# pyannote/pyannote-audio

Measured on AMD Instinct MI355X. Metric: audio-hours/sec (real-time factor) for speaker-diarization-3.1 pipeline, higher is better.
Workload: dtype f32

## Files before the change

pyannote-audio_amd/csrc/emb_resnet.hip:

```cpp
#include "common.h"

namespace pa {

constexpr int STEM_TS = 64;
constexpr int STEM_LD = STEM_TS + 3;

__global__ __launch_bounds__(256) void k_stem(const float* __restrict__ fb, int T, int F,
                                              const float* __restrict__ w9,
                                              const float* __restrict__ shift,
                                              float* __restrict__ out) {
  extern __shared__ float xs[];
  const int b = blockIdx.y, t0 = blockIdx.x * STEM_TS;
  const int tid = threadIdx.x;
  for (int i = tid; i < 2 * STEM_LD; i += 256) xs[(i < STEM_LD ? 0 : (F + 1) * STEM_LD - STEM_LD) + i] = 0.f;
  const int n = (STEM_TS + 2) * F;
  for (int i0 = 0; i0 < n; i0 += 8 * 256) {
    float v[8];
#pragma unroll
    for (int k = 0; k < 8; ++k) {
      const int i = i0 + tid + 256 * k;
      const int tt = i / F, ff = i - tt * F, t = t0 + tt - 1;
      v[k] = (i < n && t >= 0 && t < T) ? fb[((long)b * T + t) * F + ff] : 0.f;
    }
#pragma unroll
    for (int k = 0; k < 8; ++k) {
      const int i = i0 + tid + 256 * k;
      const int tt = i / F, ff = i - tt * F;
      if (i < n) xs[(ff + 1) * STEM_LD + tt] = v[k];
    }
  }
  const int q4 = (tid & 7) * 4, pl = tid >> 3;
  float w[9][4], sh[4];
#pragma unroll
  for (int k = 0; k < 9; ++k)
#pragma unroll
    for (int c = 0; c < 4; ++c) w[k][c] = w9[k * 32 + q4 + c];
#pragma unroll
  for (int c = 0; c < 4; ++c) sh[c] = shift[q4 + c];
  __syncthreads();
  float x0[2][3], x1[2][3], x2[2][3];
#pragma unroll
  for (int h = 0; h < 2; ++h)
#pragma unroll
    for (int dt = 0; dt < 3; ++dt) {
      x0[h][dt] = xs[0 * STEM_LD + pl + 32 * h + dt];
      x1[h][dt] = xs[1 * STEM_LD + pl + 32 * h + dt];
    }
  const bool ok0 = t0 + pl < T, ok1 = t0 + pl + 32 < T;
  float* o = out + ((long)b * F * T + t0 + pl) * 32 + q4;
  for (int f = 0; f < F; ++f) {
#pragma unroll
    for (int h = 0; h < 2; ++h)
#pragma unroll
      for (int dt = 0; dt < 3; ++dt) x2[h][dt] = xs[(f + 2) * STEM_LD + pl + 32 * h + dt];
    float* of = o + (long)f * T * 32;
#pragma unroll
    for (int h = 0; h < 2; ++h) {
      float acc[4];
#pragma unroll
      for (int c = 0; c < 4; ++c) acc[c] = 0.f;
#pragma unroll
      for (int dt = 0; dt < 3; ++dt)
#pragma unroll
        for (int c = 0; c < 4; ++c) acc[c] = fmaf(x0[h][dt], w[dt][c], acc[c]);
#pragma unroll
      for (int dt = 0; dt < 3; ++dt)
#pragma unroll
        for (int c = 0; c < 4; ++c) acc[c] = fmaf(x1[h][dt], w[3 + dt][c], acc[c]);
#pragma unroll
      for (int dt = 0; dt < 3; ++dt)
#pragma unroll
        for (int c = 0; c < 4; ++c) acc[c] = fmaf(x2[h][dt], w[6 + dt][c], acc[c]);
      float4 o4;
      o4.x = fmaxf(acc[0] + sh[0], 0.f);
      o4.y = fmaxf(acc[1] + sh[1], 0.f);
      o4.z = fmaxf(acc[2] + sh[2], 0.f);
      o4.w = fmaxf(acc[3] + sh[3], 0.f);
      if (h == 0 ? ok0 : ok1) *reinterpret_cast<float4*>(of + 32 * 32 * h) = o4;
    }
#pragma unroll
    for (int h = 0; h < 2; ++h)
#pragma unroll
      for (int dt = 0; dt < 3; ++dt) {
        x0[h][dt] = x1[h][dt];
        x1[h][dt] = x2[h][dt];
      }
  }
}

constexpr int CB = 16;
constexpr int CLD = CB + 4;

template <int S, int TH, int TWT>
struct ConvGeom {
  static constexpr int TW = 32 * TWT;
  static constexpr int PH = (TH - 1) * S + 3;
  static constexpr int PW = (TW - 1) * S + 3;
  static constexpr int PWH = ((TW + 1 + 3) / 8) * 8 + 4;
  static constexpr int PATCH = S == 1 ? PH * PW * CLD : PH * 2 * PWH * CLD;
};

template <int S, int TH, int TWT, int BN, bool HAS_R>
__global__ __launch_bounds__(256, 2) void k_conv3x3(const float* __restrict__ X, int H, int W, int CIN,
                                                    const float* __restrict__ Wg,
                                                    const float* __restrict__ shift,
                                                    const float* __restrict__ R, float* __restrict__ Y,
                                                    int Ho, int Wo, int COUT, int relu, int tiles_w,
                                                    int tiles_hw, int n_tiles, int total_tiles, int xranges,
                                                    int* __restrict__ counters) {
  using G = ConvGeom<S, TH, TWT>;
  constexpr int MT = TH * TWT;
  constexpr int MPW = MT / 4;
  constexpr int NT = BN / 32;
  static_assert(MT % 4 == 0, "M-tiles must split over 4 waves");
  extern __shared__ __attribute__((aligned(16))) float smem[];
  float* patch = smem;
  float* wts = smem + G::PATCH;

  const int tid = threadIdx.x, lane = tid & 63, wv = tid >> 6;
  const int li = lane & 31, kh = lane >> 5;
  constexpr int NPF4 = G::PH * G::PW * (CB / 4);
  constexpr int NP = (NPF4 + 255) / 256;
  constexpr int NWF4 = 9 * BN * (CB / 4);
  constexpr int NW = (NWF4 + 255) / 256;
  constexpr int OOB = (int)0x80000000;

  struct Tile {
    int b, n0, y0, x0;
  };
  const int num_pb = total_tiles / n_tiles;
  auto pair_of = [&](int t) {
    return xranges ? (t & 7) * ((num_pb + 7) >> 3) + (t >> 3) / n_tiles : ((t >> 3) / n_tiles) * 8 + (t & 7);
  };
  auto decode = [&](int t) {
    Tile q;
    const int pb = pair_of(t);
    q.n0 = (((t >> 3) % n_tiles)) * BN;
    const int pix = pb % tiles_hw;
    q.b = pb / tiles_hw;
    q.y0 = (pix / tiles_w) * TH;
    q.x0 = (pix % tiles_w) * G::TW;
    return q;
  };
  auto resolve = [&](const TileQueue& tqq, int r) {
    for (;;) {
      const int t = tq_resolve(tqq, r);
      if (t < 0 || pair_of(t) < num_pb) return t;
      r = tq_claim_own(tqq);
    }
  };
  u32x4 rp[NP], rw[NW];
  constexpr bool HOIST = S == 2;
  struct Offs {
    int p[NP];
  };
  int offw[NW];
#pragma unroll
  for (int e = 0; e < NW; ++e) {
    const int i = tid + 256 * e;
    const int c4 = i & 3, rn = i >> 2;
    const int tap = rn / BN, n = rn % BN;
    offw[e] = (NWF4 % 256 == 0 || i < NWF4) ? ((tap * COUT + n) * CIN + 4 * c4) * 4 : OOB;
  }
  auto tile_offsets = [&](const Tile& q, Offs& o) {
#pragma unroll
    for (int e = 0; e < NP; ++e) {
      const int i = tid + 256 * e;
      const int c4 = i & 3, pp = i >> 2;
      const int py = pp / G::PW, px = pp % G::PW;
      const int iy = q.y0 * S - 1 + py, ix = q.x0 * S - 1 + px;
      o.p[e] = ((NPF4 % 256 == 0 || i < NPF4) && iy >= 0 && iy < H && ix >= 0 && ix < W)
                   ? ((iy * W + ix) * CIN + 4 * c4) * 4
                   : OOB;
    }
  };
  auto gload = [&](const Tile& q, const Offs& o, int c0) {
    const __amdgpu_buffer_rsrc_t xsrd = __builtin_amdgcn_make_buffer_rsrc(
        const_cast<float*>(X + (long)q.b * H * W * CIN), 0, H * W * CIN * 4, 0x00020000);
    const __amdgpu_buffer_rsrc_t wsrd = __builtin_amdgcn_make_buffer_rsrc(
        const_cast<float*>(Wg + (long)q.n0 * CIN), 0, (9 * COUT - q.n0) * CIN * 4, 0x00020000);
    Offs here;
    if (!HOIST) tile_offsets(q, here);
#pragma unroll
    for (int e = 0; e < NP; ++e)
      rp[e] = __builtin_amdgcn_raw_buffer_load_b128(xsrd, HOIST ? o.p[e] : here.p[e], c0 * 4, 0);
#pragma unroll
    for (int e = 0; e < NW; ++e) rw[e] = __builtin_amdgcn_raw_buffer_load_b128(wsrd, offw[e], c0 * 4, 0);
  };
  auto lstore = [&]() {
#pragma unroll
    for (int e = 0; e < NP; ++e) {
      const int i = tid + 256 * e;
      const int c4 = i & 3, pp = i >> 2;
      const int py = pp / G::PW, px = pp % G::PW;
      int off;
      if (S == 1) off = pp * CLD + 4 * c4;
      else off = ((py * 2 + (px & 1)) * G::PWH + (px >> 1)) * CLD + 4 * c4;
      if (NPF4 % 256 == 0 || i < NPF4) *reinterpret_cast<u32x4*>(patch + off) = rp[e];
    }
#pragma unroll
    for (int e = 0; e < NW; ++e) {
      const int i = tid + 256 * e;
      if (NWF4 % 256 == 0 || i < NWF4)
        *reinterpret_cast<u32x4*>(wts + (i >> 2) * CLD + 4 * (i & 3)) = rw[e];
    }
  };

  __shared__ int s_next;
  const TileQueue tq{counters, (int)(blockIdx.x & 7), ((num_pb + 7) >> 3) * n_tiles};
  if (tid == 0) s_next = resolve(tq, tq_claim_own(tq));
  __syncthreads();
  int t = s_next;
  if (t < 0) {
    if (tid == 0) tq_done(tq, gridDim.x);
    return;
  }
  Tile cur = decode(t);
  Offs oc, on;
  if (HOIST) tile_offsets(cur, oc);
  on = oc;
  gload(cur, oc, 0);
  for (;;) {
    int ahead = 0;
    if (tid == 0) ahead = tq_claim_own(tq);
    int tn = -1;
    f32x16 acc[MPW][NT];
#pragma unroll
    for (int i = 0; i < MPW; ++i)
#pragma unroll
      for (int j = 0; j < NT; ++j)
#pragma unroll
        for (int r = 0; r < 16; ++r) acc[i][j][r] = 0.f;
    Tile nxt = cur;

    for (int c0 = 0; c0 < CIN; c0 += CB) {
      __syncthreads();
      lstore();
      if (c0 == 0 && tid == 0) s_next = resolve(tq, ahead);
      __syncthreads();
      if (c0 == 0) {
        tn = s_next;
        if (tn >= 0) {
          nxt = decode(tn);
          if (HOIST) tile_offsets(nxt, on);
        }
      }
      if (c0 + CB < CIN) gload(cur, oc, c0 + CB);
      else if (tn >= 0) gload(nxt, on, 0);
      float4 af[1][MPW][2], bf[1][NT][2];
      auto load_tap = [&](int tap, float4 (&a)[MPW][2], float4 (&bq)[NT][2]) {
        const int dy = tap / 3, dx = tap % 3;
#pragma unroll
        for (int i = 0; i < MPW; ++i) {
          const int mt = wv * MPW + i;
          const int yy = mt / TWT, xt = mt % TWT;
          int off;
          if (S == 1) off = ((yy + dy) * G::PW + 32 * xt + li + dx) * CLD;
          else off = (((yy * 2 + dy) * 2 + (dx & 1)) * G::PWH + 32 * xt + li + (dx >> 1)) * CLD;
          a[i][0] = *reinterpret_cast<const float4*>(patch + off + kh * 8);
          a[i][1] = *reinterpret_cast<const float4*>(patch + off + kh * 8 + 4);
        }
#pragma unroll
        for (int j = 0; j < NT; ++j) {
          const int off = (tap * BN + 32 * j + li) * CLD + kh * 8;
          bq[j][0] = *reinterpret_cast<const float4*>(wts + off);
          bq[j][1] = *reinterpret_cast<const float4*>(wts + off + 4);
        }
      };
      auto mfma_tap = [&](const float4 (&a)[MPW][2], const float4 (&bq)[NT][2]) {
#pragma unroll
        for (int h = 0; h < 2; ++h)
#pragma unroll
          for (int i = 0; i < MPW; ++i)
#pragma unroll
            for (int j = 0; j < NT; ++j) {
              acc[i][j] = MFMA32(a[i][h].x, bq[j][h].x, acc[i][j]);
              acc[i][j] = MFMA32(a[i][h].y, bq[j][h].y, acc[i][j]);
              acc[i][j] = MFMA32(a[i][h].z, bq[j][h].z, acc[i][j]);
              acc[i][j] = MFMA32(a[i][h].w, bq[j][h].w, acc[i][j]);
            }
      };
#pragma unroll 1
      for (int dy = 0; dy < 3; ++dy)
#pragma unroll
        for (int dx = 0; dx < 3; ++dx) {
          load_tap(dy * 3 + dx, af[0], bf[0]);
          mfma_tap(af[0], bf[0]);
        }
    }
    {
      const __amdgpu_buffer_rsrc_t ysrd = __builtin_amdgcn_make_buffer_rsrc(
          Y + (long)cur.b * Ho * Wo * COUT, 0, Ho * Wo * COUT * 4, 0x00020000);
      const __amdgpu_buffer_rsrc_t rsrd = __builtin_amdgcn_make_buffer_rsrc(
          const_cast<float*>(HAS_R ? R + (long)cur.b * Ho * Wo * COUT : Y), 0,
          Ho * Wo * COUT * 4, 0x00020000);
      constexpr int NG = MPW * NT;
      int off[2][16];
      float rv[2][16];
      auto goffs = [&](int g, int* o) {
        const int i = g / NT, j = g % NT;
        const int mt = wv * MPW + i;
        const int y = cur.y0 + mt / TWT, xbase = cur.x0 + 32 * (mt % TWT) + 4 * kh;
        const int n = cur.n0 + 32 * j + li;
#pragma unroll
        for (int r = 0; r < 16; ++r) {
          const int x = xbase + (r & 3) + 8 * (r >> 2);
          o[r] = (y < Ho && x < Wo) ? ((y * Wo + x) * COUT + n) * 4 : OOB;
        }
      };
      auto gres = [&](const int* o, float* v) {
        if (HAS_R) {
#pragma unroll
          for (int r = 0; r < 16; ++r)
            v[r] = __builtin_bit_cast(float, __builtin_amdgcn_raw_buffer_load_b32(rsrd, o[r], 0, 0));
        } else {
#pragma unroll
          for (int r = 0; r < 16; ++r) v[r] = 0.f;
        }
      };
      goffs(0, off[0]);
      gres(off[0], rv[0]);
#pragma unroll
      for (int g = 0; g < NG; ++g) {
        if (g + 1 < NG) {
          goffs(g + 1, off[(g + 1) & 1]);
          gres(off[(g + 1) & 1], rv[(g + 1) & 1]);
        }
        const int i = g / NT, j = g % NT;
        const float sh = shift[cur.n0 + 32 * j + li];
#pragma unroll
        for (int r = 0; r < 16; ++r) {
          float v = acc[i][j][r] + sh + rv[g & 1][r];
          if (relu) v = fmaxf(v, 0.f);
          __builtin_amdgcn_raw_buffer_store_b32(__builtin_bit_cast(unsigned int, v), ysrd, off[g & 1][r], 0, 0);
        }
      }
    }
    if (tn < 0) break;
    cur = nxt;
    oc = on;
  }
  if (tid == 0) tq_done(tq, gridDim.x);
}

int xcd_ranges_wanted(bool by_default);

template <int S, int TH, int TWT, int BN, bool HAS_R>
static int launch_conv_r(const float* X, int B, int H, int W, int CIN, const float* Wg,
                         const float* shift, const float* R, float* Y, int COUT, int relu,
                         hipStream_t st) {
  using G = ConvGeom<S, TH, TWT>;
  const int Ho = (H - 1) / S + 1, Wo = (W - 1) / S + 1;
  const int tiles_w = cdiv(Wo, G::TW), tiles_h = cdiv(Ho, TH);
  const size_t lds = (size_t)(G::PATCH + 9 * BN * CLD) * sizeof(float);
  constexpr int MAXDEV = 16;
  static int resident_of[MAXDEV] = {0}, per_cu_of[MAXDEV] = {0};
  int dev = 0;
  (void)hipGetDevice(&dev);
  if (dev < 0 || dev >= MAXDEV) dev = 0;
  if (!resident_of[dev]) {
    (void)hipFuncSetAttribute((const void*)k_conv3x3<S, TH, TWT, BN, HAS_R>,
                              hipFuncAttributeMaxDynamicSharedMemorySize, (int)lds);
    int cus = 256, per_cu = 2;
    (void)hipDeviceGetAttribute(&cus, hipDeviceAttributeMultiprocessorCount, dev);
    if (hipOccupancyMaxActiveBlocksPerMultiprocessor(&per_cu, k_conv3x3<S, TH, TWT, BN, HAS_R>, 256, lds) !=
            hipSuccess || per_cu < 1)
      per_cu = 2;
    resident_of[dev] = cus * per_cu;
    per_cu_of[dev] = per_cu;
  }
  const int resident = resident_of[dev] & ~7;
  const int tiles_hw = tiles_w * tiles_h, n_tiles = COUT / BN;
  const long total = (long)tiles_hw * n_tiles * B;
  const int grid = (int)(total < resident ? total : resident);
  int* counters = tile_counters();
  if (counters == nullptr) {
    set_error("pa_conv3x3: cannot allocate the tile counters");
    return 2;
  }
  hipLaunchKernelGGL((k_conv3x3<S, TH, TWT, BN, HAS_R>), dim3(grid), dim3(256), lds, st, X, H, W, CIN, Wg,
                     shift, R, Y, Ho, Wo, COUT, relu, tiles_w, tiles_hw, n_tiles, (int)total, xcd_ranges_wanted(true),
                     counters);
  return 0;
}

template <int S, int TH, int TWT, int BN>
static int launch_conv(const float* X, int B, int H, int W, int CIN, const float* Wg,
                       const float* shift, const float* R, float* Y, int COUT, int relu,
                       hipStream_t st) {
  return R != nullptr ? launch_conv_r<S, TH, TWT, BN, true>(X, B, H, W, CIN, Wg, shift, R, Y, COUT, relu, st)
                      : launch_conv_r<S, TH, TWT, BN, false>(X, B, H, W, CIN, Wg, shift, R, Y, COUT, relu, st);
}

}

extern "C" {

int pa_resnet_stem(const float* fbank, int B, int T, int F, const float* w9, const float* shift,
                   float* out, void* stream) {
  if (B <= 0) return 0;
  pa::ProfScope prof("k_stem", stream, 2.0 * B * T * F * 9 * 32, 4.0 * B * T * F * 33);
  PA_REQUIRE(F >= 1 && (size_t)(F + 2) * pa::STEM_LD * 4 <= 64 * 1024, "pa_resnet_stem: %d mel bins do not fit LDS", F);
  hipLaunchKernelGGL(pa::k_stem, dim3(pa::cdiv(T, pa::STEM_TS), B), dim3(256), (size_t)(F + 2) * pa::STEM_LD * 4,
                     (hipStream_t)stream, fbank, T, F, w9, shift, out);
  PA_CHECK_LAUNCH("pa_resnet_stem");
  return 0;
}

int pa_conv3x3(const float* X, int B, int H, int W, int cin, const float* Wg, const float* shift,
               const float* R, float* Y, int cout, int stride, int relu, void* stream) {
  if (B <= 0) return 0;
  PA_REQUIRE(cin % pa::CB == 0 && cout % 32 == 0, "pa_conv3x3: cin %% 16 and cout %% 32 required");
  hipStream_t st = (hipStream_t)stream;
  const int Ho = (H - 1) / stride + 1, Wo_ = (W - 1) / stride + 1;
  pa::ProfScope prof("k_conv3x3", stream, 2.0 * 9 * cin * cout * (double)B * Ho * Wo_,
                     4.0 * ((double)B * H * W * cin + (double)B * Ho * Wo_ * cout * (R ? 2 : 1) + 9.0 * cin * cout));
  if (stride == 1) {
    if (cout == 32) pa::launch_conv<1, 8, 1, 32>(X, B, H, W, cin, Wg, shift, R, Y, cout, relu, st);
    else if (Ho >= 32) pa::launch_conv<1, 8, 1, 64>(X, B, H, W, cin, Wg, shift, R, Y, cout, relu, st);
    else if (Ho >= 16) pa::launch_conv<1, 4, 2, 64>(X, B, H, W, cin, Wg, shift, R, Y, cout, relu, st);
    else pa::launch_conv<1, 2, 2, 64>(X, B, H, W, cin, Wg, shift, R, Y, cout, relu, st);
  } else if (stride == 2) {
    PA_REQUIRE(cout % 64 == 0, "pa_conv3x3: stride 2 needs cout %% 64 == 0");
    if (Ho >= 16) pa::launch_conv<2, 4, 1, 32>(X, B, H, W, cin, Wg, shift, R, Y, cout, relu, st);
    else pa::launch_conv<2, 2, 2, 32>(X, B, H, W, cin, Wg, shift, R, Y, cout, relu, st);
  } else {
    PA_REQUIRE(false, "pa_conv3x3: stride %d not supported", stride);
  }
  PA_CHECK_LAUNCH("pa_conv3x3");
  return 0;
}

}
```

Baseline: 1.310.

## Add dedicated stride-2 conv kernel with direct-to-LDS double-buffered loads

```diff
diff --git a/pyannote-audio_amd/csrc/emb_conv_s2.hip b/pyannote-audio_amd/csrc/emb_conv_s2.hip
--- /dev/null
+++ b/pyannote-audio_amd/csrc/emb_conv_s2.hip
@@ -0,0 +1,350 @@
+#include "common.h"
+#include "emb_conv_s2_geom.h"
+
+namespace pa {
+
+typedef __attribute__((address_space(3))) unsigned char* cs2_lds_t;
+typedef const volatile f32x4 __attribute__((address_space(3))) * cs2_lds_f32x4_ptr;
+__device__ __forceinline__ f32x4 cs2_lds_read128(cs2_lds_t p) { return *(cs2_lds_f32x4_ptr)p; }
+
+__device__ __forceinline__ void cs2_barrier() {
+  asm volatile("s_waitcnt lgkmcnt(0)" ::: "memory");
+  __builtin_amdgcn_s_barrier();
+  asm volatile("" ::: "memory");
+}
+
+#define CS2_STR2(x) #x
+#define CS2_STR(x) CS2_STR2(x)
+#define CS2_TAIL_WAIT_LIT 32
+static_assert(ConvS2Geom<4, 1>::TILE_STORES == CS2_TAIL_WAIT_LIT && ConvS2Geom<2, 2>::TILE_STORES == CS2_TAIL_WAIT_LIT,
+              "the literal of the s_waitcnt string");
+static_assert(ConvS2Geom<4, 1>::NPW <= CS2_SLOTS && ConvS2Geom<2, 2>::NPW <= CS2_SLOTS, "a slot of the MFMA run per piece");
+
+template <int IMM>
+__device__ __forceinline__ void cs2_piece(unsigned dst, int voff, __amdgpu_buffer_rsrc_t srd, int soff) {
+  asm volatile("s_add_u32 m0, %0, %1\n\ts_nop 0\n\tbuffer_load_dwordx4 %2, %3, %4 offen lds"
+               :: "s"(dst), "i"(IMM), "v"(voff), "s"(srd), "s"(soff)
+               : "memory", "scc");
+}
+__device__ __forceinline__ void cs2_piece_s(unsigned dst, int delta, int voff, __amdgpu_buffer_rsrc_t srd, int soff) {
+  asm volatile("s_add_u32 m0, %0, %1\n\ts_nop 0\n\tbuffer_load_dwordx4 %2, %3, %4 offen lds"
+               :: "s"(dst), "s"(delta), "v"(voff), "s"(srd), "s"(soff)
+               : "memory", "scc");
+}
+struct Cs2Stage {
+  __amdgpu_buffer_rsrc_t xsrd, wsrd;
+  int soff;
+  unsigned pdst, wdst;
+  int last_delta;
+};
+template <class G, int N>
+__device__ __forceinline__ void cs2_issue(const Cs2Stage& st, const int (&poff)[G::PPW], const int (&woff)[G::WPW]) {
+  if constexpr (N < G::PPW - 1) cs2_piece<4096 * N>(st.pdst, poff[N], st.xsrd, st.soff);
+  else if constexpr (N == G::PPW - 1) cs2_piece_s(st.pdst, st.last_delta, poff[N], st.xsrd, st.soff);
+  else if constexpr (N < G::NPW) cs2_piece<4096 * (N - G::PPW)>(st.wdst, woff[N - G::PPW], st.wsrd, st.soff);
+}
+template <class G>
+__device__ __forceinline__ void cs2_issue_n(const int n, const Cs2Stage& st, const int (&poff)[G::PPW],
+                                            const int (&woff)[G::WPW]) {
+  switch (n) {
+#define CS2_CASE(I) case I: cs2_issue<G, I>(st, poff, woff); break;
+    CS2_CASE(0) CS2_CASE(1) CS2_CASE(2) CS2_CASE(3) CS2_CASE(4) CS2_CASE(5) CS2_CASE(6) CS2_CASE(7) CS2_CASE(8)
+    CS2_CASE(9) CS2_CASE(10) CS2_CASE(11) CS2_CASE(12) CS2_CASE(13) CS2_CASE(14) CS2_CASE(15) CS2_CASE(16)
+    CS2_CASE(17) CS2_CASE(18) CS2_CASE(19) CS2_CASE(20) CS2_CASE(21) CS2_CASE(22) CS2_CASE(23) CS2_CASE(24)
+    CS2_CASE(25) CS2_CASE(26)
+#undef CS2_CASE
+    default: break;
+  }
+}
+
+template <int TH, int TWT, bool HAS_R>
+__global__ __launch_bounds__(256, 2) void k_conv3x3_s2(const float* __restrict__ X, int H, int W, int CIN,
+                                                       const float* __restrict__ Wg,
+                                                       const float* __restrict__ shift,
+                                                       const float* __restrict__ R, float* __restrict__ Y, int Ho,
+                                                       int Wo, int COUT, int relu, int tiles_w, int tiles_hw,
+                                                       int n_tiles, int total_tiles, int xranges,
+                                                       int* __restrict__ counters) {
+  using G = ConvS2Geom<TH, TWT>;
+  constexpr int BN = CS2_BN;
+  constexpr int OOB = CS2_OOB;
+  extern __shared__ __attribute__((aligned(16))) unsigned char smem_s2[];
+  const cs2_lds_t lds = (cs2_lds_t)smem_s2;
+  const unsigned lds0 = (unsigned)(size_t)lds;
+  int* mail = reinterpret_cast<int*>(smem_s2 + G::LDS_BYTES);
+
+  const int tid = threadIdx.x, lane = tid & 63;
+  const int slw = __builtin_amdgcn_readfirstlane(tid >> 6);
+  const int li = lane & 31, kh = lane >> 5;
+
+  struct Tile {
+    int b, n0, y0, x0;
+  };
+  const int num_pb = total_tiles / n_tiles;
+  auto pair_of = [&](int t) {
+    return xranges ? (t & 7) * ((num_pb + 7) >> 3) + (t >> 3) / n_tiles : ((t >> 3) / n_tiles) * 8 + (t & 7);
+  };
+  auto decode = [&](int t) {
+    Tile q;
+    const int pb = pair_of(t);
+    q.n0 = (((t >> 3) % n_tiles)) * BN;
+    const int pix = pb % tiles_hw;
+    q.b = pb / tiles_hw;
+    q.y0 = (pix / tiles_w) * TH;
+    q.x0 = (pix % tiles_w) * G::TW;
+    return q;
+  };
+  auto resolve = [&](const TileQueue& tqq, int r) {
+    for (;;) {
+      const int t = tq_resolve(tqq, r);
+      if (t < 0 || pair_of(t) < num_pb) return t;
+      r = tq_claim_own(tqq);
+    }
+  };
+
+  cs2_lds_t aptr[9][2];
+#pragma unroll
+  for (int tap = 0; tap < 9; ++tap)
+#pragma unroll
+    for (int h = 0; h < 2; ++h) {
+      aptr[tap][h] = lds + conv_s2_a_addr<G>(slw, li, kh, h, tap);
+      asm volatile("" : "+v"(aptr[tap][h]));
+    }
+  cs2_lds_t bptr[2];
+#pragma unroll
+  for (int h = 0; h < 2; ++h) {
+    bptr[h] = lds + G::W_BASE + conv_s2_b_addr(0, li, kh, h, 0);
+    asm volatile("" : "+v"(bptr[h]));
+  }
+  ConvS2Lane pl[G::PPW];
+#pragma unroll
+  for (int k = 0; k < G::PPW; ++k) pl[k] = conv_s2_patch_lane<G>(conv_s2_patch_piece<G>(slw, k), lane, W, CIN);
+  int woff[G::WPW];
+#pragma unroll
+  for (int k = 0; k < G::WPW; ++k) woff[k] = conv_s2_w_lane(4 * k + slw, lane, COUT, CIN);
+  const int last_delta = 1024 * (conv_s2_patch_piece<G>(slw, G::PPW - 1) - slw);
+  int poff[G::PPW];
+  auto tile_offsets = [&](const Tile& q) {
+    const int sy = 2 * q.y0 - 1, sx = 2 * q.x0 - 1, sbase = conv_s2_tile_base(q.y0, q.x0, W, CIN);
+#pragma unroll
+    for (int k = 0; k < G::PPW; ++k) poff[k] = conv_s2_patch_off(pl[k], sy, sx, sbase, H, W);
+  };
+  auto x_srd = [&](const Tile& q, bool live) {
+    return __builtin_amdgcn_make_buffer_rsrc(const_cast<float*>(X + (long)q.b * H * W * CIN), 0,
+                                             live ? H * W * CIN * 4 : 0, 0x00020000);
+  };
+  auto w_srd = [&](const Tile& q, bool live) {
+    return __builtin_amdgcn_make_buffer_rsrc(const_cast<float*>(Wg + (long)q.n0 * CIN), 0,
+                                             live ? (9 * COUT - q.n0) * CIN * 4 : 0, 0x00020000);
+  };
+  auto stage_to = [&](int to_buf, __amdgpu_buffer_rsrc_t xs, __amdgpu_buffer_rsrc_t ws, int c0) {
+    Cs2Stage st;
+    st.xsrd = xs;
+    st.wsrd = ws;
+    st.soff = c0 * 4;
+    st.pdst = lds0 + to_buf * G::PATCH_BYTES + 1024 * slw;
+    st.wdst = lds0 + G::W_BASE + to_buf * G::W_BYTES + 1024 * slw;
+    st.last_delta = __builtin_amdgcn_readfirstlane(last_delta);
+    return st;
+  };
+
+  const TileQueue tq{counters, (int)(blockIdx.x & 7), ((num_pb + 7) >> 3) * n_tiles};
+  if (tid == 0) mail[0] = resolve(tq, tq_claim_own(tq));
+  __syncthreads();
+  const int t0 = __builtin_amdgcn_readfirstlane(mail[0]);
+  if (t0 < 0) {
+    if (tid == 0) tq_done(tq, gridDim.x);
+    return;
+  }
+  Tile cur = decode(t0), nxt = cur;
+  __amdgpu_buffer_rsrc_t xcur = x_srd(cur, true), wcur = w_srd(cur, true);
+  tile_offsets(cur);
+  {
+    const Cs2Stage st = stage_to(0, xcur, wcur, 0);
+#pragma unroll
+    for (int n = 0; n < G::NPW; ++n) cs2_issue_n<G>(n, st, poff, woff);
+  }
+  int claim = 0;
+  if (tid == 0) claim = tq_claim_own(tq);
+  const int nst = CIN / CS2_CB;
+  int buf = 0, tpar = 1, tn = -1;
+  bool first_tile = true;
+
+  for (;;) {
+    f32x16 acc[2];
+#pragma unroll
+    for (int j = 0; j < 2; ++j)
+#pragma unroll
+      for (int r = 0; r < 16; ++r) acc[j][r] = 0.f;
+    for (int s = 0; s < nst; ++s) {
+      const bool last = s == nst - 1;
+      if (s == 0 && !first_tile) asm volatile("s_waitcnt vmcnt(" CS2_STR(CS2_TAIL_WAIT_LIT) ")" ::: "memory");
+      else asm volatile("s_waitcnt vmcnt(0)" ::: "memory");
+      if (last && tid == 0) mail[tpar] = resolve(tq, claim);
+      cs2_barrier();
+      Cs2Stage st;
+      auto setup = [&]() {
+        __amdgpu_buffer_rsrc_t xs = xcur, ws = wcur;
+        if (last) {
+          tn = __builtin_amdgcn_readfirstlane(mail[tpar]);
+          if (tn >= 0) {
+            nxt = decode(tn);
+            tile_offsets(nxt);
+          }
+          xs = x_srd(nxt, tn >= 0);
+          ws = w_srd(nxt, tn >= 0);
+        }
+        st = stage_to(buf ^ 1, xs, ws, last ? 0 : (s + 1) * CS2_CB);
+      };
+
+      {
+        f32x4 fa[2][2], fb[2][2][2];
+        auto rd = [&](const int tap, const int r, const int par) {
+          const int h = r / 3, w = r % 3;
+          if (w == 0) fa[par][h] = cs2_lds_read128(aptr[tap][h]);
+          else fb[par][w - 1][h] = cs2_lds_read128(bptr[h] + tap * 4096 + (w - 1) * 2048);
+        };
+#pragma unroll
+        for (int r = 0; r < 6; ++r) rd(0, r, 0);
+        __builtin_amdgcn_sched_barrier(0);
+        setup();
+        __builtin_amdgcn_sched_barrier(0);
+#pragma unroll
+        for (int tap = 0; tap < 9; ++tap) {
+          const int par = tap & 1;
+#pragma unroll
+          for (int m = 0; m < 16; ++m) {
+            const int h = m >> 3, c = (m >> 1) & 3, j = m & 1;
+            const float av = fa[par][h][c], bv = fb[par][j][h][c];
+            acc[j] = MFMA32(av, bv, acc[j]);
+            __builtin_amdgcn_sched_barrier(0);
+            if (tap + 1 < 9 && (m & 1) == 0 && m < 12) {
+              rd(tap + 1, m >> 1, par ^ 1);
+              __builtin_amdgcn_sched_barrier(0);
+            }
+            const int slot = conv_s2_slot_of(tap, m);
+            if (slot >= 0 && slot < G::NPW) {
+              cs2_issue_n<G>(slot, st, poff, woff);
+              __builtin_amdgcn_sched_barrier(0);
+            }
+          }
+        }
+      }
+      {
+        const int dp = buf ? -G::PATCH_BYTES : G::PATCH_BYTES, dw = buf ? -G::W_BYTES : G::W_BYTES;
+#pragma unroll
+        for (int tap = 0; tap < 9; ++tap)
+#pragma unroll
+          for (int h = 0; h < 2; ++h) {
+            aptr[tap][h] += dp;
+            asm volatile("" : "+v"(aptr[tap][h]));
+          }
+#pragma unroll
+        for (int h = 0; h < 2; ++h) {
+          bptr[h] += dw;
+          asm volatile("" : "+v"(bptr[h]));
+        }
+      }
+      buf ^= 1;
+    }
+    if (tid == 0 && tn >= 0) claim = tq_claim_own(tq);
+    first_tile = false;
+    {
+      const __amdgpu_buffer_rsrc_t ysrd = __builtin_amdgcn_make_buffer_rsrc(
+          Y + (long)cur.b * Ho * Wo * COUT, 0, Ho * Wo * COUT * 4, 0x00020000);
+      const __amdgpu_buffer_rsrc_t rsrd = __builtin_amdgcn_make_buffer_rsrc(
+          const_cast<float*>(HAS_R ? R + (long)cur.b * Ho * Wo * COUT : Y), 0, Ho * Wo * COUT * 4, 0x00020000);
+      const int y = cur.y0 + slw / TWT, xbase = cur.x0 + 32 * (slw % TWT) + 4 * kh;
+      int off[2][16];
+      float rv[2][16];
+      auto goffs = [&](int j, int* o) {
+        const int n = cur.n0 + 32 * j + li;
+#pragma unroll
+        for (int r = 0; r < 16; ++r) {
+          const int x = xbase + (r & 3) + 8 * (r >> 2);
+          o[r] = (y < Ho && x < Wo) ? ((y * Wo + x) * COUT + n) * 4 : OOB;
+        }
+      };
+      auto gres = [&](const int* o, float* v) {
+        if (HAS_R) {
+#pragma unroll
+          for (int r = 0; r < 16; ++r)
+            v[r] = __builtin_bit_cast(float, __builtin_amdgcn_raw_buffer_load_b32(rsrd, o[r], 0, 0));
+        } else {
+#pragma unroll
+          for (int r = 0; r < 16; ++r) v[r] = 0.f;
+        }
+      };
+      const float shv[2] = {shift[cur.n0 + li], shift[cur.n0 + 32 + li]};
+      goffs(0, off[0]);
+      gres(off[0], rv[0]);
+#pragma unroll
+      for (int j = 0; j < 2; ++j) {
+        if (j + 1 < 2) {
+          goffs(j + 1, off[(j + 1) & 1]);
+          gres(off[(j + 1) & 1], rv[(j + 1) & 1]);
+        }
+        const float sh = shv[j];
+#pragma unroll
+        for (int r = 0; r < 16; ++r) {
+          float v = acc[j][r] + sh + rv[j & 1][r];
+          if (relu) v = fmaxf(v, 0.f);
+          __builtin_amdgcn_raw_buffer_store_b32(__builtin_bit_cast(unsigned int, v), ysrd, off[j & 1][r], 0, 0);
+        }
+      }
+    }
+    if (tn < 0) break;
+    cur = nxt;
+    xcur = x_srd(cur, true);
+    wcur = w_srd(cur, true);
+    tpar ^= 1;
+  }
+  if (tid == 0) tq_done(tq, gridDim.x);
+}
+
+int xcd_ranges_wanted(bool by_default);
+
+template <int TH, int TWT, bool HAS_R>
+static int launch_conv_s2_r(const float* X, int B, int H, int W, int CIN, const float* Wg, const float* shift,
+                            const float* R, float* Y, int COUT, int relu, hipStream_t st) {
+  using G = ConvS2Geom<TH, TWT>;
+  const int Ho = (H - 1) / 2 + 1, Wo = (W - 1) / 2 + 1;
+  const int tiles_w = cdiv(Wo, G::TW), tiles_h = cdiv(Ho, TH);
+  const size_t lds = (size_t)G::LDS_BYTES + 16;
+  constexpr int MAXDEV = 16;
+  static int resident_of[MAXDEV] = {0};
+  int dev = 0;
+  (void)hipGetDevice(&dev);
+  if (dev < 0 || dev >= MAXDEV) dev = 0;
+  if (!resident_of[dev]) {
+    (void)hipFuncSetAttribute((const void*)k_conv3x3_s2<TH, TWT, HAS_R>, hipFuncAttributeMaxDynamicSharedMemorySize,
+                              (int)lds);
+    int cus = 256;
+    (void)hipDeviceGetAttribute(&cus, hipDeviceAttributeMultiprocessorCount, dev);
+    resident_of[dev] = cus;
+  }
+  const int resident = resident_of[dev] & ~7;
+  const int tiles_hw = tiles_w * tiles_h, n_tiles = COUT / CS2_BN;
+  const long total = (long)tiles_hw * n_tiles * B;
+  const int grid = (int)(total < resident ? total : resident);
+  int* counters = tile_counters();
+  if (counters == nullptr) {
+    set_error("pa_conv3x3: cannot allocate the tile counters");
+    return 2;
+  }
+  hipLaunchKernelGGL((k_conv3x3_s2<TH, TWT, HAS_R>), dim3(grid), dim3(256), lds, st, X, H, W, CIN, Wg, shift, R, Y, Ho,
+                     Wo, COUT, relu, tiles_w, tiles_hw, n_tiles, (int)total, xcd_ranges_wanted(true), counters);
+  return 0;
+}
+
+int launch_conv_s2(const float* X, int B, int H, int W, int CIN, const float* Wg, const float* shift, const float* R,
+                   float* Y, int COUT, int relu, hipStream_t st) {
+  const int Ho = (H - 1) / 2 + 1;
+  if (Ho >= 16)
+    return R != nullptr ? launch_conv_s2_r<4, 1, true>(X, B, H, W, CIN, Wg, shift, R, Y, COUT, relu, st)
+                        : launch_conv_s2_r<4, 1, false>(X, B, H, W, CIN, Wg, shift, R, Y, COUT, relu, st);
+  return R != nullptr ? launch_conv_s2_r<2, 2, true>(X, B, H, W, CIN, Wg, shift, R, Y, COUT, relu, st)
+                      : launch_conv_s2_r<2, 2, false>(X, B, H, W, CIN, Wg, shift, R, Y, COUT, relu, st);
+}
+
+}
diff --git a/pyannote-audio_amd/csrc/emb_conv_s2_geom.h b/pyannote-audio_amd/csrc/emb_conv_s2_geom.h
--- /dev/null
+++ b/pyannote-audio_amd/csrc/emb_conv_s2_geom.h
@@ -0,0 +1,90 @@
+#pragma once
+
+namespace pa {
+
+constexpr int CS2_CB = 16;
+constexpr int CS2_BN = 64;
+constexpr int CS2_OOB = (int)0x80000000;
+
+template <int TH_, int TWT_>
+struct ConvS2Geom {
+  static constexpr int TH = TH_, TWT = TWT_, TW = 32 * TWT_;
+  static constexpr int PH = 2 * TH + 1, PW = 2 * TW + 1;
+  static constexpr int PWH = TW + 1;
+  static constexpr int PENT = PH * 2 * PWH;
+  static constexpr int PPIECES = (PENT + 15) / 16;
+  static constexpr int WPIECES = 9 * CS2_BN / 16;
+  static constexpr int PPW = (PPIECES + 3) / 4;
+  static constexpr int WPW = WPIECES / 4;
+  static constexpr int NPW = PPW + WPW;
+  static constexpr int PATCH_BYTES = PPIECES * 1024;
+  static constexpr int W_BYTES = WPIECES * 1024;
+  static constexpr int W_BASE = 2 * PATCH_BYTES;
+  static constexpr int LDS_BYTES = 2 * (PATCH_BYTES + W_BYTES);
+  static constexpr int TILE_STORES = 2 * 16;
+  static_assert(TH * TWT == 4, "one M-tile per wave, four waves");
+  static_assert(WPIECES % 4 == 0 && PPW * 4 >= PPIECES, "pieces split over four waves");
+  static_assert(8 * 4096 + 2048 < 65536, "ds_read immediates of a B fragment: tap and N-tile");
+  static_assert(LDS_BYTES + 64 <= 160 * 1024, "two stages in LDS");
+};
+
+__device__ __forceinline__ int conv_s2_swz(int e) { return (e >> 2) & 3; }
+
+template <class G>
+__device__ __forceinline__ int conv_s2_patch_piece(int w, int k) {
+  const int i = 4 * k + w;
+  return i < G::PPIECES ? i : G::PPIECES - 1;
+}
+
+struct ConvS2Lane {
+  int rel, py, px;
+};
+constexpr int CS2_NO_COLUMN = 0x20000000;
+template <class G>
+__device__ __forceinline__ ConvS2Lane conv_s2_patch_lane(int piece, int lane, int W, int CIN) {
+  const int sl = 64 * piece + lane;
+  const int e = sl >> 2, q = (sl & 3) ^ conv_s2_swz(e);
+  const int plane = e / G::PWH, col = e % G::PWH;
+  const int py = plane >> 1, px = 2 * col + (plane & 1);
+  const bool real = e < G::PENT && px < G::PW;
+  ConvS2Lane L;
+  L.rel = ((py * W + px) * CIN + 4 * q) * 4;
+  L.py = py;
+  L.px = real ? px : CS2_NO_COLUMN;
+  return L;
+}
+__device__ __forceinline__ int conv_s2_tile_base(int y0, int x0, int W, int CIN) {
+  return ((2 * y0 - 1) * W + 2 * x0 - 1) * CIN * 4;
+}
+__device__ __forceinline__ int conv_s2_patch_off(const ConvS2Lane& L, int sy, int sx, int sbase, int H, int W) {
+  const bool ok = (unsigned)(L.py + sy) < (unsigned)H && (unsigned)(L.px + sx) < (unsigned)W;
+  return ok ? sbase + L.rel : CS2_OOB;
+}
+__device__ __forceinline__ int conv_s2_w_lane(int piece, int lane, int COUT, int CIN) {
+  const int sl = 64 * piece + lane;
+  const int e = sl >> 2, q = (sl & 3) ^ conv_s2_swz(e);
+  const int tap = e >> 6, n = e & 63;
+  return ((tap * COUT + n) * CIN + 4 * q) * 4;
+}
+
+template <class G>
+__device__ __forceinline__ int conv_s2_a_entry(int mt, int li, int tap) {
+  const int dy = tap / 3, dx = tap % 3;
+  const int yy = mt / G::TWT, xt = mt % G::TWT;
+  return ((2 * yy + dy) * 2 + (dx & 1)) * G::PWH + 32 * xt + li + (dx >> 1);
+}
+__device__ __forceinline__ int conv_s2_slot_addr(int e, int q) { return e * 64 + ((q ^ conv_s2_swz(e)) << 4); }
+template <class G>
+__device__ __forceinline__ int conv_s2_a_addr(int mt, int li, int kh, int h, int tap) {
+  return conv_s2_slot_addr(conv_s2_a_entry<G>(mt, li, tap), 2 * kh + h);
+}
+__device__ __forceinline__ int conv_s2_b_addr(int j, int li, int kh, int h, int tap) {
+  return conv_s2_slot_addr(tap * 64 + 32 * j + li, 2 * kh + h);
+}
+
+constexpr int CS2_SLOTS = 9 * 3;
+__device__ __forceinline__ int conv_s2_slot_of(int tap, int m) {
+  return (m == 3 || m == 9 || m == 15) ? tap * 3 + (m - 3) / 6 : -1;
+}
+
+}
diff --git a/pyannote-audio_amd/csrc/emb_resnet.hip b/pyannote-audio_amd/csrc/emb_resnet.hip
--- a/pyannote-audio_amd/csrc/emb_resnet.hip
+++ b/pyannote-audio_amd/csrc/emb_resnet.hip
@@ -91,16 +91,15 @@
 constexpr int CB = 16;
 constexpr int CLD = CB + 4;
 
-template <int S, int TH, int TWT>
+template <int TH, int TWT>
 struct ConvGeom {
   static constexpr int TW = 32 * TWT;
-  static constexpr int PH = (TH - 1) * S + 3;
-  static constexpr int PW = (TW - 1) * S + 3;
-  static constexpr int PWH = ((TW + 1 + 3) / 8) * 8 + 4;
-  static constexpr int PATCH = S == 1 ? PH * PW * CLD : PH * 2 * PWH * CLD;
+  static constexpr int PH = TH + 2;
+  static constexpr int PW = TW + 2;
+  static constexpr int PATCH = PH * PW * CLD;
 };
 
-template <int S, int TH, int TWT, int BN, bool HAS_R>
+template <int TH, int TWT, int BN, bool HAS_R>
 __global__ __launch_bounds__(256, 2) void k_conv3x3(const float* __restrict__ X, int H, int W, int CIN,
                                                     const float* __restrict__ Wg,
                                                     const float* __restrict__ shift,
@@ -108,7 +107,7 @@
                                                     int Ho, int Wo, int COUT, int relu, int tiles_w,
                                                     int tiles_hw, int n_tiles, int total_tiles, int xranges,
                                                     int* __restrict__ counters) {
-  using G = ConvGeom<S, TH, TWT>;
+  using G = ConvGeom<TH, TWT>;
   constexpr int MT = TH * TWT;
   constexpr int MPW = MT / 4;
   constexpr int NT = BN / 32;
@@ -150,7 +149,6 @@
     }
   };
   u32x4 rp[NP], rw[NW];
-  constexpr bool HOIST = S == 2;
   struct Offs {
     int p[NP];
   };
@@ -168,22 +166,21 @@
       const int i = tid + 256 * e;
       const int c4 = i & 3, pp = i >> 2;
       const int py = pp / G::PW, px = pp % G::PW;
-      const int iy = q.y0 * S - 1 + py, ix = q.x0 * S - 1 + px;
+      const int iy = q.y0 - 1 + py, ix = q.x0 - 1 + px;
       o.p[e] = ((NPF4 % 256 == 0 || i < NPF4) && iy >= 0 && iy < H && ix >= 0 && ix < W)
                    ? ((iy * W + ix) * CIN + 4 * c4) * 4
                    : OOB;
     }
   };
-  auto gload = [&](const Tile& q, const Offs& o, int c0) {
+  auto gload = [&](const Tile& q, int c0) {
     const __amdgpu_buffer_rsrc_t xsrd = __builtin_amdgcn_make_buffer_rsrc(
         const_cast<float*>(X + (long)q.b * H * W * CIN), 0, H * W * CIN * 4, 0x00020000);
     const __amdgpu_buffer_rsrc_t wsrd = __builtin_amdgcn_make_buffer_rsrc(
         const_cast<float*>(Wg + (long)q.n0 * CIN), 0, (9 * COUT - q.n0) * CIN * 4, 0x00020000);
     Offs here;
-    if (!HOIST) tile_offsets(q, here);
-#pragma unroll
-    for (int e = 0; e < NP; ++e)
-      rp[e] = __builtin_amdgcn_raw_buffer_load_b128(xsrd, HOIST ? o.p[e] : here.p[e], c0 * 4, 0);
+    tile_offsets(q, here);
+#pragma unroll
+    for (int e = 0; e < NP; ++e) rp[e] = __builtin_amdgcn_raw_buffer_load_b128(xsrd, here.p[e], c0 * 4, 0);
 #pragma unroll
     for (int e = 0; e < NW; ++e) rw[e] = __builtin_amdgcn_raw_buffer_load_b128(wsrd, offw[e], c0 * 4, 0);
   };
@@ -192,11 +189,7 @@
     for (int e = 0; e < NP; ++e) {
       const int i = tid + 256 * e;
       const int c4 = i & 3, pp = i >> 2;
-      const int py = pp / G::PW, px = pp % G::PW;
-      int off;
-      if (S == 1) off = pp * CLD + 4 * c4;
-      else off = ((py * 2 + (px & 1)) * G::PWH + (px >> 1)) * CLD + 4 * c4;
-      if (NPF4 % 256 == 0 || i < NPF4) *reinterpret_cast<u32x4*>(patch + off) = rp[e];
+      if (NPF4 % 256 == 0 || i < NPF4) *reinterpret_cast<u32x4*>(patch + pp * CLD + 4 * c4) = rp[e];
     }
 #pragma unroll
     for (int e = 0; e < NW; ++e) {
@@ -216,10 +209,7 @@
     return;
   }
   Tile cur = decode(t);
-  Offs oc, on;
-  if (HOIST) tile_offsets(cur, oc);
-  on = oc;
-  gload(cur, oc, 0);
+  gload(cur, 0);
   for (;;) {
     int ahead = 0;
     if (tid == 0) ahead = tq_claim_own(tq);
@@ -240,13 +230,10 @@
       __syncthreads();
       if (c0 == 0) {
         tn = s_next;
-        if (tn >= 0) {
-          nxt = decode(tn);
-          if (HOIST) tile_offsets(nxt, on);
-        }
+        if (tn >= 0) nxt = decode(tn);
       }
-      if (c0 + CB < CIN) gload(cur, oc, c0 + CB);
-      else if (tn >= 0) gload(nxt, on, 0);
+      if (c0 + CB < CIN) gload(cur, c0 + CB);
+      else if (tn >= 0) gload(nxt, 0);
       float4 af[1][MPW][2], bf[1][NT][2];
       auto load_tap = [&](int tap, float4 (&a)[MPW][2], float4 (&bq)[NT][2]) {
         const int dy = tap / 3, dx = tap % 3;
@@ -254,9 +241,7 @@
         for (int i = 0; i < MPW; ++i) {
           const int mt = wv * MPW + i;
           const int yy = mt / TWT, xt = mt % TWT;
-          int off;
-          if (S == 1) off = ((yy + dy) * G::PW + 32 * xt + li + dx) * CLD;
-          else off = (((yy * 2 + dy) * 2 + (dx & 1)) * G::PWH + 32 * xt + li + (dx >> 1)) * CLD;
+          const int off = ((yy + dy) * G::PW + 32 * xt + li + dx) * CLD;
           a[i][0] = *reinterpret_cast<const float4*>(patch + off + kh * 8);
           a[i][1] = *reinterpret_cast<const float4*>(patch + off + kh * 8 + 4);
         }
@@ -338,19 +323,20 @@
     }
     if (tn < 0) break;
     cur = nxt;
-    oc = on;
   }
   if (tid == 0) tq_done(tq, gridDim.x);
 }
 
 int xcd_ranges_wanted(bool by_default);
-
-template <int S, int TH, int TWT, int BN, bool HAS_R>
+int launch_conv_s2(const float* X, int B, int H, int W, int CIN, const float* Wg, const float* shift, const float* R,
+                   float* Y, int COUT, int relu, hipStream_t st);
+
+template <int TH, int TWT, int BN, bool HAS_R>
 static int launch_conv_r(const float* X, int B, int H, int W, int CIN, const float* Wg,
                          const float* shift, const float* R, float* Y, int COUT, int relu,
                          hipStream_t st) {
-  using G = ConvGeom<S, TH, TWT>;
-  const int Ho = (H - 1) / S + 1, Wo = (W - 1) / S + 1;
+  using G = ConvGeom<TH, TWT>;
+  const int Ho = H, Wo = W;
   const int tiles_w = cdiv(Wo, G::TW), tiles_h = cdiv(Ho, TH);
   const size_t lds = (size_t)(G::PATCH + 9 * BN * CLD) * sizeof(float);
   constexpr int MAXDEV = 16;
@@ -359,11 +345,11 @@
   (void)hipGetDevice(&dev);
   if (dev < 0 || dev >= MAXDEV) dev = 0;
   if (!resident_of[dev]) {
-    (void)hipFuncSetAttribute((const void*)k_conv3x3<S, TH, TWT, BN, HAS_R>,
+    (void)hipFuncSetAttribute((const void*)k_conv3x3<TH, TWT, BN, HAS_R>,
                               hipFuncAttributeMaxDynamicSharedMemorySize, (int)lds);
     int cus = 256, per_cu = 2;
     (void)hipDeviceGetAttribute(&cus, hipDeviceAttributeMultiprocessorCount, dev);
-    if (hipOccupancyMaxActiveBlocksPerMultiprocessor(&per_cu, k_conv3x3<S, TH, TWT, BN, HAS_R>, 256, lds) !=
+    if (hipOccupancyMaxActiveBlocksPerMultiprocessor(&per_cu, k_conv3x3<TH, TWT, BN, HAS_R>, 256, lds) !=
             hipSuccess || per_cu < 1)
       per_cu = 2;
     resident_of[dev] = cus * per_cu;
@@ -378,18 +364,18 @@
     set_error("pa_conv3x3: cannot allocate the tile counters");
     return 2;
   }
-  hipLaunchKernelGGL((k_conv3x3<S, TH, TWT, BN, HAS_R>), dim3(grid), dim3(256), lds, st, X, H, W, CIN, Wg,
+  hipLaunchKernelGGL((k_conv3x3<TH, TWT, BN, HAS_R>), dim3(grid), dim3(256), lds, st, X, H, W, CIN, Wg,
                      shift, R, Y, Ho, Wo, COUT, relu, tiles_w, tiles_hw, n_tiles, (int)total, xcd_ranges_wanted(true),
                      counters);
   return 0;
 }
 
-template <int S, int TH, int TWT, int BN>
+template <int TH, int TWT, int BN>
 static int launch_conv(const float* X, int B, int H, int W, int CIN, const float* Wg,
                        const float* shift, const float* R, float* Y, int COUT, int relu,
                        hipStream_t st) {
-  return R != nullptr ? launch_conv_r<S, TH, TWT, BN, true>(X, B, H, W, CIN, Wg, shift, R, Y, COUT, relu, st)
-                      : launch_conv_r<S, TH, TWT, BN, false>(X, B, H, W, CIN, Wg, shift, R, Y, COUT, relu, st);
+  return R != nullptr ? launch_conv_r<TH, TWT, BN, true>(X, B, H, W, CIN, Wg, shift, R, Y, COUT, relu, st)
+                      : launch_conv_r<TH, TWT, BN, false>(X, B, H, W, CIN, Wg, shift, R, Y, COUT, relu, st);
 }
 
 }
@@ -416,14 +402,13 @@
   pa::ProfScope prof("k_conv3x3", stream, 2.0 * 9 * cin * cout * (double)B * Ho * Wo_,
                      4.0 * ((double)B * H * W * cin + (double)B * Ho * Wo_ * cout * (R ? 2 : 1) + 9.0 * cin * cout));
   if (stride == 1) {
-    if (cout == 32) pa::launch_conv<1, 8, 1, 32>(X, B, H, W, cin, Wg, shift, R, Y, cout, relu, st);
-    else if (Ho >= 32) pa::launch_conv<1, 8, 1, 64>(X, B, H, W, cin, Wg, shift, R, Y, cout, relu, st);
-    else if (Ho >= 16) pa::launch_conv<1, 4, 2, 64>(X, B, H, W, cin, Wg, shift, R, Y, cout, relu, st);
-    else pa::launch_conv<1, 2, 2, 64>(X, B, H, W, cin, Wg, shift, R, Y, cout, relu, st);
+    if (cout == 32) pa::launch_conv<8, 1, 32>(X, B, H, W, cin, Wg, shift, R, Y, cout, relu, st);
+    else if (Ho >= 32) pa::launch_conv<8, 1, 64>(X, B, H, W, cin, Wg, shift, R, Y, cout, relu, st);
+    else if (Ho >= 16) pa::launch_conv<4, 2, 64>(X, B, H, W, cin, Wg, shift, R, Y, cout, relu, st);
+    else pa::launch_conv<2, 2, 64>(X, B, H, W, cin, Wg, shift, R, Y, cout, relu, st);
   } else if (stride == 2) {
     PA_REQUIRE(cout % 64 == 0, "pa_conv3x3: stride 2 needs cout %% 64 == 0");
-    if (Ho >= 16) pa::launch_conv<2, 4, 1, 32>(X, B, H, W, cin, Wg, shift, R, Y, cout, relu, st);
-    else pa::launch_conv<2, 2, 2, 32>(X, B, H, W, cin, Wg, shift, R, Y, cout, relu, st);
+    if (pa::launch_conv_s2(X, B, H, W, cin, Wg, shift, R, Y, cout, relu, st) != 0) return 2;
   } else {
     PA_REQUIRE(false, "pa_conv3x3: stride %d not supported", stride);
   }
```

Measured after the change: 1.328, median of 6. 1.4% higher.
